# NVIDIA/nv-wavenet

Hardware: AMD Instinct MI355X
Metric: samples/sec (all GPUs) in real time (every utterance >= 24 kHz) and max real-time batch @24kHz, R64/S256/A256 20L fp16 (higher is better)
Workload: dtype f16; 1 GPU; C3: R=64 S=256 A=256 L=20 maxDilation=512 fp16, autoregressive generation at steady state (each step = samples 640..895 of every utterance: all dilated taps live, all rings wrapped; the steps re-run that sample range -- same launch, same memory traffic -- so from the second step on the rings hold the previous step's values: a timing workload, not one long utterance); batch_per_gpu=12288, global_batch=12288, parallelism=batch-sharded x1, final RCCL all_gather

## Files before the change

### nv_wavenet_amd/csrc/wn_kernels.hpp

```cpp
#pragma once

#include <hip/hip_runtime.h>
#include <utility>
#include <stdint.h>

#include <type_traits>

#include "wn_experiments.hpp"

namespace wn {

#define WN_DEV __device__ __forceinline__

typedef _Float16 half8 __attribute__((ext_vector_type(8)));
typedef _Float16 half4 __attribute__((ext_vector_type(4)));
typedef float floatx4 __attribute__((ext_vector_type(4)));
typedef unsigned int uintx4 __attribute__((ext_vector_type(4)));
typedef unsigned int uintx2 __attribute__((ext_vector_type(2)));

template <bool F16> struct Prec;
template <> struct Prec<true> {
    using elem = _Float16;
    using frag = half8;
    using quad = half4;
// ... 579 lines not shown

WN_DEV float fma_mix_lo(unsigned h2, float acc) {
    float d;
    asm("v_fma_mix_f32 %0, %1, 1.0, %2 op_sel_hi:[1,0,0]" : "=v"(d) : "v"(h2), "v"(acc));
    return d;
}
WN_DEV float fma_mix_hi(unsigned h2, float acc) {
    float d;
    asm("v_fma_mix_f32 %0, %1, 1.0, %2 op_sel:[1,0,0] op_sel_hi:[1,0,0]" : "=v"(d) : "v"(h2), "v"(acc));
    return d;
}
template <bool F16> WN_DEV void cond_add(floatx4* a, typename Prec<F16>::frag c, const typename Prec<F16>::frag* selA) {
    if constexpr (F16) {
#if WN_COND_VALU
        (void)selA;
        const uintx4 q = __builtin_bit_cast(uintx4, c);
        a[0][0] = fma_mix_lo(q[0], a[0][0]);
        a[0][1] = fma_mix_hi(q[0], a[0][1]);
        a[0][2] = fma_mix_lo(q[1], a[0][2]);
        a[0][3] = fma_mix_hi(q[1], a[0][3]);
        a[1][0] = fma_mix_lo(q[2], a[1][0]);
        a[1][1] = fma_mix_hi(q[2], a[1][1]);
        a[1][2] = fma_mix_lo(q[3], a[1][2]);
        a[1][3] = fma_mix_hi(q[3], a[1][3]);
#else
#pragma unroll
        for (int tt = 0; tt < Prec<F16>::TPF; tt++) a[tt] = mma(selA[tt], c, a[tt]);
#endif
    } else {
        (void)selA;
#pragma unroll
        for (int e = 0; e < Prec<F16>::EPL; e++) a[e >> 2][e & 3] += (float)c[e];
    }
}

template <bool F16, int R, int S, int A, int BT, bool EMBLDS, bool DUMP = true, int RAW = 0, bool LR = false>
#ifdef WN_EXP_TWO_WG
__global__ __launch_bounds__((Cfg<F16, R, S, A, BT>::THREADS), (BT == 1 ? 2 : 1)) void wavenet_wg(const Params p) {
#else
__global__ __launch_bounds__((Cfg<F16, R, S, A, BT>::THREADS), 1) void wavenet_wg(const Params p) {
#endif
    constexpr bool FEAT = RAW == 3;
    constexpr int KFC = FEAT ? feat_kfc<F16>() : 0;
    using C = Cfg<F16, R, S, A, BT, KFC>;
    using P = Prec<F16>;
    using frag = typename P::frag;
    using quad = typename P::quad;
    using elem = typename P::elem;
    constexpr int PF = C::PF, FLW = C::FLW, FHW = C::FHW, NW = C::NW;
    constexpr int RT = C::RT, HTW = C::HTW, STW = C::STW, ATW = C::ATW;
    constexpr int KF_R = C::KF_R, KF_S = C::KF_S, KF_A = C::KF_A;

    extern __shared__ __attribute__((aligned(16))) char lds[];
    char* const xbuf = lds + C::OFF_X;
    char* const hbuf = lds + C::OFF_H;
    char* const skbuf = lds + C::OFF_SK;
    char* const zsbuf = lds + C::OFF_ZS;
    float* const lgbuf = (float*)(lds + C::OFF_LG);
    int* const ybuf = (int*)(lds + C::OFF_Y);
    char* const xpbuf = lds + C::OFF_XP;
    float* const biasLds = (float*)(lds + C::OFF_BIAS);

    static_assert(RAW == 0 || RAW == 1 || (RAW == 2 && F16) || RAW == 3, "RAW: 0 packed, 1 fp32 in place, 2 fp16 in place (fp16 engine), 3 features");
    if (p.gate != nullptr && __builtin_nontemporal_load(p.gate) == 0u) return;

    const int tid = threadIdx.x;
    const int lane = tid & 63;
    const int w = __builtin_amdgcn_readfirstlane(tid >> 6);
    const int g = lane >> 4, j = lane & 15;
    const int L = p.numLayers;
    const int tile0 = p.tileBase + blockIdx.x * BT;
    if (p.clk != nullptr && blockIdx.x == 0 && tid == 0) {
        p.clk[0] = __builtin_amdgcn_s_memtime();
        p.clk[1] = __builtin_amdgcn_s_memrealtime();
    }

    int ub[BT];
    bool uvalid[BT];
#pragma unroll
    for (int bt = 0; bt < BT; bt++) {
        const int b = (tile0 + bt) * 16 + j;
        uvalid[bt] = b < p.batch;
        ub[bt] = uvalid[bt] ? b : p.batch - 1;
    }
    const int su = tid / C::LPU, sq = tid % C::LPU;

    constexpr int BLS = DUMP ? C::BIAS_L : C::BIAS_LN;
    if constexpr (DUMP) {
        const int nb = L * C::BIAS_L + 2 * A;
        for (int i = tid; i < nb; i += C::THREADS) biasLds[i] = p.bias[i];
        __syncthreads();
        for (int s0 = tid; s0 < S; s0 += C::THREADS) {
            float run = biasLds[3 * R + s0];
            for (int l = 1; l < L; l++) {
                run += biasLds[l * C::BIAS_L + 3 * R + s0];
                biasLds[l * C::BIAS_L + 3 * R + s0] = run;
            }
        }
    } else {
        for (int i = tid; i < L * C::BIAS_LN; i += C::THREADS) biasLds[i] = p.bias[(i / C::BIAS_LN) * C::BIAS_L + i % C::BIAS_LN];
        for (int i = tid; i < 2 * A; i += C::THREADS) biasLds[L * C::BIAS_LN + S + i] = p.bias[L * C::BIAS_L + i];
        for (int s0 = tid; s0 < S; s0 += C::THREADS) {
            float run = p.bias[3 * R + s0];
            for (int l = 1; l < L; l++) run += p.bias[l * C::BIAS_L + 3 * R + s0];
            biasLds[L * C::BIAS_LN + s0] = run;
        }
    }
    const float* const skipBiasSum = DUMP ? biasLds + (L - 1) * C::BIAS_L + 3 * R : biasLds + L * C::BIAS_LN;
    const float* const headBias = biasLds + (C::biasFloats(L, DUMP) - 2 * A);

    const unsigned laneOff = (unsigned)lane * 16u;
    const char* const wbase = (const char*)p.wblob + (size_t)w * C::waveStreamFrags(L) * 1024;
    const char* const whead = wbase + C::headOffsetFrags(L) * 1024;
    const elem* embPrev = (const elem*)p.embPrev;
    const elem* embCur = (const elem*)p.embCur;
    if constexpr (EMBLDS) {
        elem* const embLds = (elem*)(biasLds + C::biasFloats(L, DUMP));
        const floatx4* s0 = (const floatx4*)p.embCur;
        const floatx4* s1 = (const floatx4*)p.embPrev;
        constexpr int CH = (int)(A * R * sizeof(elem) / 16);
        for (int i = tid; i < CH; i += C::THREADS) {
            ((floatx4*)embLds)[i] = s0[i];
            if (p.embLds > 1) ((floatx4*)embLds)[CH + i] = s1[i];
        }
        embCur = embLds;
        if (p.embLds > 1) embPrev = embLds + A * R;
        __syncthreads();
    }

    int yPrev[BT], yCur[BT];
    floatx4 ep[BT][HTW];
#pragma unroll
    for (int bt = 0; bt < BT; bt++) {
        yPrev[bt] = p.yInPrev[ub[bt]];
        yCur[bt] = p.yInCur[ub[bt]];
#pragma unroll
        for (int i = 0; i < HTW; i++)
            ep[bt][i] = quad_to_f32(*(const quad*)(embPrev + (size_t)yPrev[bt] * R + (w + NW * i) * 16 + g * 4));
    }

    constexpr bool ws_pin = F16 && !(RAW == 1 && BT == 2);
    WStream<F16, PF, ws_pin> ws;
    const rsrc_t rsW = make_rsrc(wbase);
#pragma unroll
    for (int i = 0; i < PF; i++) ws.buf[i] = buf_load<frag, WN_W_AUX>(rsW, laneOff + (unsigned)(i & 3) * 1024u, (unsigned)(i & ~3) * 1024u);

    constexpr int HR = C::HR, HS = C::HS;
    frag hw[HR ? HR : 1];
    if constexpr (HR > 0) {
#pragma unroll
        for (int i = 0; i < HR; i++) hw[i] = *(const frag*)(whead + (size_t)C::headFrag(HS + i) * 1024 + laneOff);
    }

    constexpr int XPW = C::XPW;
    frag xpA[BT][XPW], xpB[BT][XPW];
    constexpr int CR = (RAW == 1 && F16) ? 2 * C::COND_FR : C::COND_FR;
    frag cdA[BT][CR], cdB[BT][CR];
    constexpr int KFCR = FEAT ? KFC : 1;
    frag cfCur[BT][KFCR], cfNext[BT][KFCR];
    const size_t featStride = (size_t)p.tiles * KFC * 1024;
    const char* const featMine = (const char*)p.feat + (size_t)tile0 * KFC * 1024;
    auto load_feat = [&](int tn, frag (&dst)[BT][KFCR]) {
        const int tc = tn < p.condSamples ? tn : p.condSamples - 1;
        const rsrc_t rsF = make_rsrc(featMine + (size_t)tc * featStride);
#pragma unroll
        for (int bt = 0; bt < BT; bt++)
#pragma unroll
            for (int k = 0; k < KFC; k++)
                dst[bt][k] = buf_load<frag, WN_FEAT_AUX>(rsF, laneOff + (unsigned)(k & 3) * 1024u, (unsigned)((bt * KFC + (k & ~3)) * 1024));
    };
    const size_t condStride = (size_t)p.tiles * NW * C::COND_FR * 1024;
    const char* const condMine = (const char*)p.cond + ((size_t)tile0 * NW + w) * C::COND_FR * 1024;
    const size_t ringTile = (size_t)p.ringSlots * KF_R * 1024;
    char* const ringMine = (char*)p.ring + (size_t)tile0 * ringTile;
    const rsrc_t rsRing = make_rsrc(ringMine);
    const unsigned ringTileB = (unsigned)ringTile;
    const int ldsD = LR ? p.ldsRingD : 0;
    char* const ringLds = lds + C::ringSlotOffset(0, (int)C::ldsBytes(L, EMBLDS ? p.embLds : 0, DUMP));
    const char* condNext = condMine + (size_t)p.initSample * L * condStride;
    constexpr unsigned RAWE = RAW == 2 ? 2u : 4u;
    const size_t rawRow = (size_t)p.maxBatch * (2 * R) * RAWE;
    unsigned rawOff[BT];
#pragma unroll
    for (int bt = 0; bt < BT; bt++) rawOff[bt] = ((unsigned)ub[bt] * (unsigned)(2 * R) + (unsigned)g * 4u) * RAWE;
    auto prefetch = [&](int tn, int ln, Dil dl, frag (&xd)[BT][XPW], frag (&cdd)[BT][CR]) {
        if (ln >= L) { ln -= L; tn += 1; }
        const unsigned slot = (unsigned)(dl.off + (tn & (dl.d - 1)));
        const unsigned rp0 = slot * (unsigned)(KF_R * 1024);
        const rsrc_t rsCond = make_rsrc(condNext);
        condNext += condStride;
        if (dl.d > ldsD) {
#pragma unroll
            for (int i = 0; i < XPW; i++) {
                const int k = w + NW * i;
                if (k < KF_R) {
#pragma unroll
                    for (int bt = 0; bt < BT; bt++)
                        xd[bt][i] = buf_load<frag, WN_RING_LD_AUX>(rsRing, laneOff, rp0 + (unsigned)bt * ringTileB + (unsigned)k * 1024u);
                }
            }
        }
#pragma unroll
        for (int bt = 0; bt < BT; bt++) {
            if constexpr (FEAT) {
            } else if constexpr (RAW != 0) {
                const int tc = tn < p.condSamples ? tn : p.condSamples - 1;
                const rsrc_t rsRaw = make_rsrc((const char*)p.condRaw + ((size_t)tc * L + ln) * rawRow);
                auto slotOff = [&](int it) { return (unsigned)((w + NW * (it >> 1) + (it & 1) * RT) * 16) * RAWE; };
                if constexpr (RAW == 1) {
#pragma unroll
                    for (int it = 0; it < 2 * HTW; it++) cdd[bt][it] = buf_load<frag, WN_RAW_AUX>(rsRaw, rawOff[bt], slotOff(it));
                } else {
#pragma unroll
                    for (int k = 0; k < HTW; k++) {
                        const uintx2 qa = __builtin_amdgcn_raw_buffer_load_b64(rsRaw, rawOff[bt], slotOff(2 * k), WN_RAW_AUX);
                        const uintx2 qb = __builtin_amdgcn_raw_buffer_load_b64(rsRaw, rawOff[bt], slotOff(2 * k + 1), WN_RAW_AUX);
                        cdd[bt][k] = __builtin_bit_cast(frag, uintx4{qa[0], qa[1], qb[0], qb[1]});
                    }
                }
            } else {
#pragma unroll
                for (int k = 0; k < C::COND_FR; k++)
                    cdd[bt][k] = buf_load<frag, WN_COND_AUX>(rsCond, laneOff + (unsigned)(k & 3) * 1024u,
                                                   (unsigned)((bt * NW * C::COND_FR + (k & ~3)) * 1024));
            }
        }
    };
    auto ring_lds_copy = [&](auto TOLDS) {
        constexpr bool toLds = decltype(TOLDS)::value;
        if (ldsD <= 0) return;
        Dil dl = dil_first();
        for (int l = 0; l < L; l++) {
            if (dl.d <= ldsD) {
                const int rows = dl.d * BT * KF_R;
                for (int r = w; r < rows; r += NW) {
                    const int sl = r / (BT * KF_R), bt = (r / KF_R) % BT, k = r % KF_R;
                    const unsigned hb = (unsigned)(dl.off + sl) * (unsigned)(KF_R * 1024) + (unsigned)bt * ringTileB + (unsigned)k * 1024u;
                    char* const lp = ringLds + (size_t)(dl.lds + sl) * C::RING_SLOT + ((bt * KF_R + k) * 64 + lane) * 16;
                    if constexpr (toLds) *(frag*)lp = buf_load<frag, WN_RING_LD_AUX>(rsRing, laneOff, hb);
                    else buf_store<frag, WN_RING_ST_AUX>(rsRing, laneOff, hb, *(const frag*)lp);
                }
            }
            dl = dil_next(dl, p.maxDilation, false, ldsD);
        }
    };
    ring_lds_copy(std::true_type{});
    prefetch(p.initSample, 0, p.dil[0], xpA, cdA);
    prefetch(p.initSample, 1, p.dil[1], xpB, cdB);
    auto publish_xp = [&](const frag (&xpN)[BT][XPW], const Dil dN) {
        if (dN.d <= ldsD) return;
#pragma unroll
        for (int i = 0; i < XPW; i++) {
            const int k = w + NW * i;
            if (k < KF_R) {
#pragma unroll
                for (int bt = 0; bt < BT; bt++) *(frag*)(xpbuf + ((bt * KF_R + k) * 64 + lane) * 16) = xpN[bt][i];
            }
        }
    };
    auto tap_image = [&](const Dil dN, int tn) -> const char* {
        return dN.d <= ldsD ? ringLds + (size_t)(dN.lds + (tn & (dN.d - 1))) * C::RING_SLOT : xpbuf;
    };
    publish_xp(xpA, p.dil[0]);

    __syncthreads();

#ifdef WN_TIMING
    unsigned long long tacc[12] = {0};
    unsigned long long tmark = 0;
#define WN_TMARK(i)                                                        \
    {                                                                      \
        unsigned long long _n = __builtin_amdgcn_s_memtime();              \
        asm volatile("s_waitcnt lgkmcnt(0)" ::: "memory");                 \
        tacc[i] += _n - tmark;                                             \
        tmark = _n;                                                        \
    }
#else
#define WN_TMARK(i)
#endif
    frag selA[P::TPF];
#pragma unroll
    for (int tt = 0; tt < P::TPF; tt++)
#pragma unroll
        for (int e = 0; e < P::EPL; e++)
            selA[tt][e] = (elem)(((e >> 2) == tt && g * 4 + (e & 3) == j) ? 1.0f : 0.0f);
    floatx4 acc[BT][2 * HTW];
    {
        frag xp[BT][KF_R];
#pragma unroll
        for (int bt = 0; bt < BT; bt++) {
            lds_get_frags<F16, KF_R>(tap_image(p.dil[0], p.initSample) + bt * KF_R * 1024, lane, xp[bt]);
#pragma unroll
            for (int i = 0; i < HTW; i++) {
                acc[bt][2 * i] = *(const floatx4*)(biasLds + (w + NW * i) * 16 + g * 4);
                acc[bt][2 * i + 1] = *(const floatx4*)(biasLds + (w + NW * i + RT) * 16 + g * 4);
            }
        }
        if constexpr (FEAT) {
            load_feat(p.initSample, cfNext);
#pragma unroll
            for (int bt = 0; bt < BT; bt++)
#pragma unroll
                for (int k = 0; k < KFC; k++) cfCur[bt][k] = agpr_operand<F16>(cfNext[bt][k]);
            gemm_direct<F16, BT, 2 * HTW, KFC>(wbase + C::streamPos(0, C::O_COND, L) * 1024, laneOff, acc, cfCur);
            load_feat(p.initSample + 1, cfNext);
#pragma unroll
            for (int bt = 0; bt < BT; bt++)
#pragma unroll
                for (int k = 0; k < KFC; k++) asm volatile("" ::"v"(cfNext[bt][k]));
        } else {
#pragma unroll
            for (int bt = 0; bt < BT; bt++)
#pragma unroll
                for (int k = 0; k < C::COND_FR; k++) cond_add<F16>(&acc[bt][k * P::TPF], cond_frag<F16, RAW>(cdA[bt], k), selA);
        }
        gemm_direct<F16, BT, 2 * HTW, KF_R>(wbase + C::streamPos(0, C::O_PREV, L) * 1024, laneOff, acc, xp);
    }
    float sscale[FEAT ? BT : 1];
    if constexpr (FEAT) {
#pragma unroll
        for (int bt = 0; bt < BT; bt++) {
            int sb = (tile0 + bt) * 16 + su;
            sb = sb < p.batch ? sb : p.batch - 1;
            sscale[bt] = p.softScale != nullptr ? p.softScale[sb] : kLog2e;
        }
    }
    const int tEnd = p.initSample + p.count;
    for (int t = p.initSample; t < tEnd; t++) {
        const bool dumpNow = DUMP && p.dump && (t == tEnd - 1);

        float selv[BT];
        if (!p.useRng) {
#pragma unroll
            for (int bt = 0; bt < BT; bt++) {
                int sb = (tile0 + bt) * 16 + su;
                sb = sb < p.batch ? sb : p.batch - 1;
                selv[bt] = p.sel[(size_t)t * p.maxBatch + sb];
            }
        }

        WN_TMARK(11)
        floatx4 x[BT][HTW];
#pragma unroll
        for (int bt = 0; bt < BT; bt++) {
#pragma unroll
            for (int i = 0; i < HTW; i++) {
                const int tile = w + NW * i;
                floatx4 ec = quad_to_f32(*(const quad*)(embCur + (size_t)yCur[bt] * R + tile * 16 + g * 4));
                floatx4 v = ep[bt][i] + ec;
                if (p.tanhEmbed) {
#pragma unroll
                    for (int r = 0; r < 4; r++) v[r] = tanh_t<F16>(v[r]);
                }
                x[bt][i] = v;
                lds_put_tile<F16>(xbuf + bt * KF_R * 1024, tile, lane, v);
            }
#pragma unroll
            for (int i = 0; i < HTW; i++)
                ep[bt][i] = quad_to_f32(*(const quad*)(embPrev + (size_t)yCur[bt] * R + (w + NW * i) * 16 + g * 4));
        }
        wg_barrier();
        WN_TMARK(0)

        floatx4 skip[BT][STW];
#pragma unroll
        for (int bt = 0; bt < BT; bt++)
#pragma unroll
            for (int i = 0; i < STW; i++) skip[bt][i] = floatx4{0.f, 0.f, 0.f, 0.f};

        frag hb[BT][KF_R];
        frag xb[BT][KF_R];
#pragma unroll
        for (int bt = 0; bt < BT; bt++) lds_get_frags<F16, KF_R>(xbuf + bt * KF_R * 1024, lane, xb[bt]);
        auto layer = [&](auto withSkip, const int l, const Dil dl, const Dil dN, const Dil dl2, frag (&xpC)[BT][XPW],
                         frag (&cdC)[BT][CR], const frag (&xpN)[BT][XPW], const frag (&cdN)[BT][CR]) {
            constexpr bool SKIP = decltype(withSkip)::value;
            constexpr int PB = SKIP ? 0 : FLW;
            const int wl = SKIP ? (l - 1) * FLW : 0;
            const float* bl = biasLds + l * BLS;
            const int lN = l + 1 < L ? l + 1 : 0;
            const float* blN = biasLds + lN * BLS;
            const int d = dl.d;

            WN_TMARK(1)
            gemm_b<F16, PF, 0, BT, 2 * HTW, KF_R>(ws, rsW, SKIP ? C::P_CUR : C::P_CUR0 - PB, wl, 0, laneOff, acc, xb);
            const bool ringInLds = d <= ldsD;
            frag xkeep[BT][XPW];
            if (!ringInLds) {
                const unsigned rp = (unsigned)(dl.off + (t & (d - 1))) * (unsigned)(KF_R * 1024);
#pragma unroll
                for (int k = 0; k < KF_R; k++)
                    if (k % NW == w) {
#pragma unroll
                        for (int bt = 0; bt < BT; bt++)
                            buf_store<frag, WN_RING_ST_AUX>(rsRing, laneOff + (unsigned)(k & 3) * 1024u,
                                               rp + (unsigned)bt * ringTileB + (unsigned)(k & ~3) * 1024u, xb[bt][k]);
                    }
            } else {
#pragma unroll
                for (int k = 0; k < KF_R; k++)
                    if (k % NW == w) {
#pragma unroll
                        for (int bt = 0; bt < BT; bt++) xkeep[bt][k / NW] = xb[bt][k];
                    }
            }
            if constexpr (!SKIP) prefetch(t, l + 2, dl2, xpC, cdC);
            __builtin_amdgcn_sched_barrier(0);
            WN_TMARK(2)

            floatx4 accN[FEAT ? BT : 1][2 * HTW];
            if constexpr (FEAT) {
#pragma unroll
                for (int bt = 0; bt < BT; bt++)
#pragma unroll
                    for (int i = 0; i < HTW; i++) {
                        accN[bt][2 * i] = *(const floatx4*)(blN + (w + NW * i) * 16 + g * 4);
                        accN[bt][2 * i + 1] = *(const floatx4*)(blN + (w + NW * i + RT) * 16 + g * 4);
                    }
            }
            if constexpr (FEAT) {
                constexpr int NS = BT * HTW * 2 * 5;
                constexpr int NFS = SKIP ? STW * KF_R : 0, NFC = C::FW_COND;
                constexpr int NM = (NFS + NFC) * BT;
                constexpr int G0S = STW >= 4 ? 4 : STW, G0C = 2 * HTW >= 4 ? 4 : 2 * HTW;
                constexpr bool EARLY = PF > 1;
                floatx2 ea, eb, ra, rb, hp;
                floatx4 hv;
                auto stage = [&](auto SI) {
                    constexpr int s = decltype(SI)::value, pr = s / 5, st = s % 5;
                    constexpr int bt = pr / (2 * HTW), i = (pr / 2) % HTW, r = (pr & 1) * 2;
                    gate_stage<F16, st>(acc[bt][2 * i][r], acc[bt][2 * i][r + 1], acc[bt][2 * i + 1][r], acc[bt][2 * i + 1][r + 1],
                                        ea, eb, ra, rb, hp);
                    if constexpr (st == 4) {
                        hv[r] = hp[0];
                        hv[r + 1] = hp[1];
                        if constexpr (r == 2) lds_put_tile<F16>(hbuf + bt * KF_R * 1024, w + NW * i, lane, hv);
                    }
                    __builtin_amdgcn_sched_barrier(0);
                };
                static_for<NFS + NFC>([&](auto FI) {
                    constexpr int fi = decltype(FI)::value;
                    constexpr bool isSkip = fi < NFS;
                    constexpr int q = isSkip ? fi : fi - NFS, G0 = isSkip ? G0S : G0C, KFq = isSkip ? KF_R : KFC;
                    constexpr int kf = (q / G0) % KFq, mt = (q / (G0 * KFq)) * G0 + q % G0;
                    constexpr int pos = isSkip ? C::P_SKIP + q : C::P_COND - PB + q;
                    constexpr int posPrev = (fi - 1 < NFS) ? C::P_SKIP + fi - 1 : C::P_COND - PB + fi - 1 - NFS;
                    frag a[1];
                    take_group<F16, PF, ws_pin, 1>(ws, pos, a);
                    if constexpr (EARLY && fi > 0) refill_group<F16, PF, 0, ws_pin, 1>(ws, rsW, posPrev, wl, 0, laneOff);
                    static_for<BT>([&](auto BI) {
                        constexpr int bt = decltype(BI)::value, m = fi * BT + bt;
                        if constexpr (isSkip) skip[bt][mt] = mma(a[0], hb[bt][kf], skip[bt][mt]);
                        else accN[bt][mt] = mma(a[0], cfCur[bt][kf], accN[bt][mt]);
                        __builtin_amdgcn_sched_barrier(0);
                        static_for_range<m * NS / NM, (m + 1) * NS / NM>(stage);
                    });
                    if constexpr (!EARLY || fi == NFS + NFC - 1) refill_group<F16, PF, 0, ws_pin, 1>(ws, rsW, pos, wl, 0, laneOff);
                    if constexpr (SKIP && fi == (NFS + NFC) * WN_REQ_AT_FEAT / 8) {
                        prefetch(t, l + 2, dl2, xpC, cdC);
                        __builtin_amdgcn_sched_barrier(0);
                    }
                });
                if (l == L - 2) {
                    asm volatile("");
#pragma unroll
                    for (int bt = 0; bt < BT; bt++)
#pragma unroll
                        for (int k = 0; k < KFC; k++) cfCur[bt][k] = agpr_operand<F16>(cfNext[bt][k]);
                }
                if constexpr (SKIP) {
                    if (dumpNow) {
                        const float* bp = biasLds + (l - 1) * C::BIAS_L + 3 * R;
#pragma unroll
                        for (int bt = 0; bt < BT; bt++) {
                            if (!uvalid[bt]) continue;
#pragma unroll
                            for (int i = 0; i < STW; i++)
                                *(floatx4*)(p.skipOut + ((size_t)(l - 1) * p.maxBatch + ub[bt]) * S + (w + NW * i) * 16 + g * 4) =
                                    skip[bt][i] + *(const floatx4*)(bp + (w + NW * i) * 16 + g * 4);
                        }
                    }
                }
            } else {
                constexpr int NS = BT * HTW * 2 * 5;
                constexpr int NM = SKIP ? STW * KF_R * BT : 0;
                floatx2 ea, eb, ra, rb, hp;
                floatx4 hv;
                auto stage = [&](auto SI) {
                    constexpr int s = decltype(SI)::value, pr = s / 5, st = s % 5;
                    constexpr int bt = pr / (2 * HTW), i = (pr / 2) % HTW, r = (pr & 1) * 2;
                    gate_stage<F16, st>(acc[bt][2 * i][r], acc[bt][2 * i][r + 1], acc[bt][2 * i + 1][r], acc[bt][2 * i + 1][r + 1],
                                        ea, eb, ra, rb, hp);
                    if constexpr (st == 4) {
                        hv[r] = hp[0];
                        hv[r + 1] = hp[1];
                        if constexpr (r == 2) lds_put_tile<F16>(hbuf + bt * KF_R * 1024, w + NW * i, lane, hv);
                    }
                    __builtin_amdgcn_sched_barrier(0);
                };
                if constexpr (SKIP) {
                    constexpr int G0 = STW >= 4 ? 4 : STW, G = take_g(G0, PF);
                    static_for<STW * KF_R / G>([&](auto GI) {
                        constexpr int gi = decltype(GI)::value, q = gi * G;
                        constexpr int kf = (q / G0) % KF_R, mg = q / (G0 * KF_R), mi0 = q % G0;
                        frag a[G];
                        take_group<F16, PF, ws_pin, G>(ws, C::P_SKIP + gi * G, a);
                        constexpr bool EARLY = PF > G;
                        if constexpr (EARLY && gi > 0) refill_group<F16, PF, 0, ws_pin, G>(ws, rsW, C::P_SKIP + (gi - 1) * G, wl, 0, laneOff);
                        static_for<G * BT>([&](auto MI) {
                            constexpr int mi = decltype(MI)::value / BT, bt = decltype(MI)::value % BT;
                            constexpr int mt = mg * G0 + mi0 + mi, m = (q + mi) * BT + bt;
                            skip[bt][mt] = mma(a[mi], hb[bt][kf], skip[bt][mt]);
                            __builtin_amdgcn_sched_barrier(0);
                            static_for_range<m * NS / NM, (m + 1) * NS / NM>(stage);
                        });
                        if constexpr (!EARLY || gi == STW * KF_R / G - 1) refill_group<F16, PF, 0, ws_pin, G>(ws, rsW, C::P_SKIP + gi * G, wl, 0, laneOff);
                        if constexpr (gi == (STW * KF_R / G) * WN_REQ_AT / 8) {
                            prefetch(t, l + 2, dl2, xpC, cdC);
                            __builtin_amdgcn_sched_barrier(0);
                        }
                    });
                    if (dumpNow) {
                        const float* bp = biasLds + (l - 1) * C::BIAS_L + 3 * R;
#pragma unroll
                        for (int bt = 0; bt < BT; bt++) {
                            if (!uvalid[bt]) continue;
#pragma unroll
                            for (int i = 0; i < STW; i++)
                                *(floatx4*)(p.skipOut + ((size_t)(l - 1) * p.maxBatch + ub[bt]) * S + (w + NW * i) * 16 + g * 4) =
                                    skip[bt][i] + *(const floatx4*)(bp + (w + NW * i) * 16 + g * 4);
                        }
                    }
                } else {
                    static_for<NS>(stage);
                }
            }
            WN_TMARK(3)
            wg_barrier();
            WN_TMARK(4)
#pragma unroll
            for (int bt = 0; bt < BT; bt++) lds_get_frags<F16, KF_R>(hbuf + bt * KF_R * 1024, lane, hb[bt]);
            if (ringInLds) {
                char* const sl = ringLds + (size_t)(dl.lds + (t & (d - 1))) * C::RING_SLOT;
#pragma unroll
                for (int i = 0; i < XPW; i++) {
                    const int k = w + NW * i;
                    if (k < KF_R) {
#pragma unroll
                        for (int bt = 0; bt < BT; bt++) *(frag*)(sl + ((bt * KF_R + k) * 64 + lane) * 16) = xkeep[bt][i];
                    }
                }
            }

            floatx4 xa[BT][HTW];
#pragma unroll
            for (int bt = 0; bt < BT; bt++)
#pragma unroll
                for (int i = 0; i < HTW; i++)
                    xa[bt][i] = *(const floatx4*)(bl + 2 * R + (w + NW * i) * 16 + g * 4) + x[bt][i];
#pragma unroll
            for (int bt = 0; bt < BT; bt++)
#pragma unroll
                for (int i = 0; i < HTW; i++) {
                    if constexpr (FEAT) {
                        acc[bt][2 * i] = accN[bt][2 * i];
                        acc[bt][2 * i + 1] = accN[bt][2 * i + 1];
                    } else {
                        acc[bt][2 * i] = *(const floatx4*)(blN + (w + NW * i) * 16 + g * 4);
                        acc[bt][2 * i + 1] = *(const floatx4*)(blN + (w + NW * i + RT) * 16 + g * 4);
                    }
                }

            gemm_b<F16, PF, 0, BT, HTW, KF_R>(ws, rsW, C::P_RES - PB, wl, 0, laneOff, xa, hb);
#pragma unroll
            for (int bt = 0; bt < BT; bt++)
#pragma unroll
                for (int i = 0; i < HTW; i++) {
                    x[bt][i] = xa[bt][i];
                    lds_put_tile<F16>(xbuf + bt * KF_R * 1024, w + NW * i, lane, xa[bt][i]);
                }
            publish_xp(xpN, dN);
            __builtin_amdgcn_sched_barrier(0);
            WN_TMARK(5)
            if constexpr (FEAT) {
            } else {
#pragma unroll
                for (int bt = 0; bt < BT; bt++)
#pragma unroll
                    for (int k = 0; k < C::COND_FR; k++) cond_add<F16>(&acc[bt][k * P::TPF], cond_frag<F16, RAW>(cdN[bt], k), selA);
            }
            if (dumpNow) {
#pragma unroll
                for (int bt = 0; bt < BT; bt++) {
                    if (!uvalid[bt]) continue;
#pragma unroll
                    for (int i = 0; i < HTW; i++)
                        *(floatx4*)(p.xtOut + ((size_t)l * p.maxBatch + ub[bt]) * R + (w + NW * i) * 16 + g * 4) = x[bt][i];
                }
            }
            __builtin_amdgcn_sched_barrier(0);
            WN_TMARK(6)
            wg_barrier();
            WN_TMARK(7)
            frag xp[BT][KF_R];
            const char* const tapImg = tap_image(dN, l + 1 < L ? t : t + 1);
#pragma unroll
            for (int bt = 0; bt < BT; bt++) lds_get_frags<F16, KF_R>(tapImg + bt * KF_R * 1024, lane, xp[bt]);
#pragma unroll
            for (int bt = 0; bt < BT; bt++) lds_get_frags<F16, KF_R>(xbuf + bt * KF_R * 1024, lane, xb[bt]);
            __builtin_amdgcn_sched_barrier(0);
            gemm_b<F16, PF, 0, BT, 2 * HTW, KF_R>(ws, rsW, C::P_PREV - PB, wl, 0, laneOff, acc, xp);
        };
        {
            Dil da = dil_first(), db = dil_next(da, p.maxDilation, L == 1, ldsD), dc = dil_next(db, p.maxDilation, L == 2, ldsD);
            auto adv = [&](int l) { da = db; db = dc; dc = dil_next(dc, p.maxDilation, l + 3 == L, ldsD); };
            layer(std::false_type{}, 0, da, db, dc, xpA, cdA, xpB, cdB);
            adv(0);
            int l = 1;
            for (; l + 1 < L; l += 2) {
                layer(std::true_type{}, l, da, db, dc, xpB, cdB, xpA, cdA);
                adv(l);
                layer(std::true_type{}, l + 1, da, db, dc, xpA, cdA, xpB, cdB);
                adv(l + 1);
            }
            if (l < L) layer(std::true_type{}, l, da, db, dc, xpB, cdB, xpA, cdA);
            if (L & 1) {
#pragma unroll
                for (int bt = 0; bt < BT; bt++) {
#pragma unroll
                    for (int i = 0; i < XPW; i++) {
                        const frag tmp = xpA[bt][i];
                        xpA[bt][i] = xpB[bt][i];
                        xpB[bt][i] = tmp;
                    }
#pragma unroll
                    for (int k = 0; k < CR; k++) {
                        const frag tmp = cdA[bt][k];
                        cdA[bt][k] = cdB[bt][k];
                        cdB[bt][k] = tmp;
                    }
                }
            }
        }
        gemm_b<F16, PF, 0, BT, STW, KF_R>(ws, rsW, C::P_CUR, (L - 1) * FLW, 0, laneOff, skip, hb);

#pragma unroll
        for (int bt = 0; bt < BT; bt++)
#pragma unroll
            for (int i = 0; i < STW; i++) {
                floatx4 v = skip[bt][i] + *(const floatx4*)(skipBiasSum + (w + NW * i) * 16 + g * 4);
#pragma unroll
                for (int r = 0; r < 4; r++) v[r] = __builtin_fmaxf(v[r], 0.f);
                lds_put_tile<F16>(skbuf + bt * KF_S * 1024, w + NW * i, lane, v);
                if (dumpNow && uvalid[bt])
                    *(floatx4*)(p.skipOut + ((size_t)(L - 1) * p.maxBatch + ub[bt]) * S + (w + NW * i) * 16 + g * 4) = v;
            }
        wg_barrier();
        floatx4 zs[BT][ATW];
        if constexpr (HS != 0 && KF_S * BT * 4 > WN_ZS_B_REGS) {
#pragma unroll
            for (int bt = 0; bt < BT; bt++)
#pragma unroll
                for (int i = 0; i < ATW; i++) zs[bt][i] = *(const floatx4*)(headBias + (w + NW * i) * 16 + g * 4);
            gemm_ldsb_b<F16, PF, C::HSP, BT, ATW, KF_S>(ws, rsW, C::O_ZS, L * FLW, 0, laneOff, zs, skbuf, lane);
            skip_frags<F16, PF, C::HSP, ws_pin, C::PAD1>(ws, rsW, C::FW_ZS, L * FLW, 0, laneOff);
        } else {
            frag sb[BT][KF_S];
#pragma unroll
            for (int bt = 0; bt < BT; bt++) {
                lds_get_frags<F16, KF_S>(skbuf + bt * KF_S * 1024, lane, sb[bt]);
#pragma unroll
                for (int i = 0; i < ATW; i++) zs[bt][i] = *(const floatx4*)(headBias + (w + NW * i) * 16 + g * 4);
            }
            if constexpr (HS == 0) gemm_res<F16, BT, ATW, KF_S>(hw, 0, zs, sb);
            else {
                gemm_b<F16, PF, C::HSP, BT, ATW, KF_S>(ws, rsW, C::O_ZS, L * FLW, 0, laneOff, zs, sb);
                skip_frags<F16, PF, C::HSP, ws_pin, C::PAD1>(ws, rsW, C::FW_ZS, L * FLW, 0, laneOff);
            }
        }
#pragma unroll
        for (int bt = 0; bt < BT; bt++)
#pragma unroll
            for (int i = 0; i < ATW; i++) {
#pragma unroll
                for (int r = 0; r < 4; r++) zs[bt][i][r] = __builtin_fmaxf(zs[bt][i][r], 0.f);
                lds_put_tile<F16>(zsbuf + bt * KF_A * 1024, w + NW * i, lane, zs[bt][i]);
                if (dumpNow && uvalid[bt])
                    *(floatx4*)(p.zs + (size_t)ub[bt] * A + (w + NW * i) * 16 + g * 4) = zs[bt][i];
            }
        wg_barrier();
        floatx4 za[BT][ATW];
        {
#pragma unroll
            for (int bt = 0; bt < BT; bt++)
#pragma unroll
                for (int i = 0; i < ATW; i++)
                    za[bt][i] = *(const floatx4*)(headBias + A + (w + NW * i) * 16 + g * 4);
            auto draw_selectors = [&]() {
                if (!p.useRng) return;
                if constexpr (C::LPU == 16 && BT > 1) {
                    const int q = sq < BT ? sq : 0;
                    int sb = (tile0 + q) * 16 + su;
                    sb = sb < p.batch ? sb : p.batch - 1;
                    const float mine = philox_selector(p.rngKey0, p.rngKey1, (unsigned)t, (unsigned)sb);
                    selv[0] = dpp_f<0x150>(mine);
                    if constexpr (BT > 1) selv[1] = dpp_f<0x151>(mine);
                    if constexpr (BT > 2) selv[2] = dpp_f<0x152>(mine);
                    if constexpr (BT > 3) selv[3] = dpp_f<0x153>(mine);
                } else {
#pragma unroll
                    for (int bt = 0; bt < BT; bt++) {
                        int sb = (tile0 + bt) * 16 + su;
                        sb = sb < p.batch ? sb : p.batch - 1;
                        selv[bt] = philox_selector(p.rngKey0, p.rngKey1, (unsigned)t, (unsigned)sb);
                    }
                }
            };
            if constexpr (C::ZA_B_FROM_LDS) {
                static_assert(HR == 0, "the LDS-streamed head is for the large, non-resident heads");
                draw_selectors();
                gemm_ldsb_b<F16, PF, C::HSP, BT, ATW, KF_A>(ws, rsW, C::O_ZA, L * FLW, 0, laneOff, za, zsbuf, lane);
            } else {
                frag zb[BT][KF_A];
#pragma unroll
                for (int bt = 0; bt < BT; bt++) lds_get_frags<F16, KF_A>(zsbuf + bt * KF_A * 1024, lane, zb[bt]);
                draw_selectors();
                if constexpr (HR >= C::FW_ZA) gemm_res<F16, BT, ATW, KF_A>(hw, C::FW_ZS - HS, za, zb);
                else gemm_b<F16, PF, C::HSP, BT, ATW, KF_A>(ws, rsW, C::O_ZA, L * FLW, 0, laneOff, za, zb);
            }
        }
        if constexpr (C::ALIAS_LG) wg_barrier();
        constexpr int LGT = C::LGT;
        auto put_logits = [&](auto PASS) {
            constexpr int pass = decltype(PASS)::value;
#pragma unroll
            for (int bl = 0; bl < LGT; bl++)
#pragma unroll
                for (int i = 0; i < ATW; i++) {
                    const int bt = pass * LGT + bl;
                    *(floatx4*)(lgbuf + (bl * 16 + j) * C::LROW + (w + NW * i) * 16 + g * 4) = za[bt][i];
                    if (dumpNow && uvalid[bt])
                        *(floatx4*)(p.za + (size_t)ub[bt] * A + (w + NW * i) * 16 + g * 4) = za[bt][i];
                }
        };
        put_logits(std::integral_constant<int, 0>{});
        WN_TMARK(8)
        if constexpr (HS == FHW) {
            skip_frags<F16, PF, C::HSP, ws_pin, C::PAD2>(ws, rsW, C::O_ZA + C::FW_ZA, L * FLW, 0, laneOff);
        }
        if constexpr (FEAT) load_feat(t + 2, cfNext);
        wg_barrier();
        WN_TMARK(9)

        static_for<BT / LGT>([&](auto PASS) {
            constexpr int pass = decltype(PASS)::value;
            if constexpr (pass > 0) {
                wg_barrier();
                put_logits(PASS);
                wg_barrier();
            }
#pragma unroll
            for (int bl = 0; bl < LGT; bl++) {
                const int bt = pass * LGT + bl;
                float e[C::RPL];
                float total;
                const float* lrow = lgbuf + (bl * 16 + su) * C::LROW + sq * C::RPL;
                int pick;
                if constexpr (FEAT) pick = softmax_pick<A, C::LPU, C::RPL>(lrow, sq, lane, selv[bt], e, total, sscale[bt]);
                else pick = softmax_pick<A, C::LPU, C::RPL>(lrow, sq, lane, selv[bt], e, total);
                const int sb = (tile0 + bt) * 16 + su;
                if (sq == 0) {
                    ybuf[bt * 16 + su] = pick;
                    if (sb < p.batch) p.yOut[(size_t)sb * p.numSamples + t] = pick;
                }
                if (dumpNow && sb < p.batch) {
                    const float inv = 1.0f / total;
#pragma unroll
                    for (int i = 0; i < C::RPL / 4; i++)
                        *(floatx4*)(p.p + (size_t)sb * A + sq * C::RPL + i * 4) =
                            floatx4{e[i * 4] * inv, e[i * 4 + 1] * inv, e[i * 4 + 2] * inv, e[i * 4 + 3] * inv};
                }
            }
        });
        wg_barrier();
#pragma unroll
        for (int bt = 0; bt < BT; bt++) {
            yPrev[bt] = yCur[bt];
// ... 343 lines not shown
```

Before: 328.7 million samples/s.

## Restructure dilation ring bookkeeping into per-wave row ownership with precomputed ring entries

Replaces the per-layer Dil slot arithmetic with a RingEnt struct that precomputes the slot offset, LDS tap pointer and whether the ring lives in LDS. Each wave now owns whole rows across the batch tiles (NROW = BT*KF_R spread over waves) for prefetch, publish and ring store. For small R the ring store and load always go through a buffer resource whose record count is zero when the ring is LDS-resident, which removes branches but issues masked global ops. Own rows are read back from xbuf instead of being kept in registers, trading register pressure for extra LDS reads.

Result: no change. 330.4 million samples/s, median of 6 (+0.5%).

```diff
diff --git a/nv_wavenet_amd/csrc/wn_kernels.hpp b/nv_wavenet_amd/csrc/wn_kernels.hpp
--- a/nv_wavenet_amd/csrc/wn_kernels.hpp
+++ b/nv_wavenet_amd/csrc/wn_kernels.hpp
@@ -755,8 +755,11 @@
         for (int i = 0; i < HR; i++) hw[i] = *(const frag*)(whead + (size_t)C::headFrag(HS + i) * 1024 + laneOff);
     }
 
-    constexpr int XPW = C::XPW;
-    frag xpA[BT][XPW], xpB[BT][XPW];
+    constexpr int NROW = BT * KF_R, RPW = (NROW + NW - 1) / NW;
+    constexpr bool OWN_EARLY = R <= 128;
+    constexpr unsigned ROWB = (unsigned)(KF_R * 1024);
+    const bool lastRow = NROW % NW == 0 || w + NW * (RPW - 1) < NROW;
+    frag xpA[RPW], xpB[RPW];
     constexpr int CR = (RAW == 1 && F16) ? 2 * C::COND_FR : C::COND_FR;
     frag cdA[BT][CR], cdB[BT][CR];
     constexpr int KFCR = FEAT ? KFC : 1;
@@ -779,29 +782,62 @@
     const rsrc_t rsRing = make_rsrc(ringMine);
     const unsigned ringTileB = (unsigned)ringTile;
     const int ldsD = LR ? p.ldsRingD : 0;
-    char* const ringLds = lds + C::ringSlotOffset(0, (int)C::ldsBytes(L, EMBLDS ? p.embLds : 0, DUMP));
+    const unsigned ringLdsOff = (unsigned)C::ringSlotOffset(0, (int)C::ldsBytes(L, EMBLDS ? p.embLds : 0, DUMP));
+    char* const ringLds = lds + ringLdsOff;
+    const unsigned rowLds = (unsigned)w * 1024u + laneOff;
+    unsigned rowHbm[RPW];
+#pragma unroll
+    for (int i = 0; i < RPW; i++) {
+        const int r = w + NW * i;
+        rowHbm[i] = BT == 1 ? rowLds : laneOff + (unsigned)(r / KF_R) * ringTileB + (unsigned)(r % KF_R) * 1024u;
+    }
+    auto row_soff = [&](unsigned slot, int i) { return BT == 1 ? slot + (unsigned)(i * NW * 1024) : slot; };
+    struct RingEnt {
+        int mask;
+        unsigned hbm;
+        char* ldsAcc;
+        int far;
+        unsigned slot;
+        char* tap;
+        WN_DEV bool inLds() const { return LR && far < 0; }
+        WN_DEV int records() const { return LR ? ~(far >> 31) : -1; }
+    };
+    auto ring_rsrc = [&](const RingEnt e) { return __builtin_amdgcn_make_buffer_rsrc((void*)ringMine, 0, e.records(), 0x00020000); };
+    auto ent_make = [&](int d, unsigned hbm, char* ldsAcc, int tn) {
+        RingEnt e;
+        e.mask = d - 1, e.hbm = hbm, e.ldsAcc = ldsAcc;
+        e.far = e.mask - ldsD;
+        const unsigned ph = (unsigned)(tn & e.mask);
+        e.slot = hbm + ph * ROWB;
+        e.tap = e.inLds() ? ldsAcc + ph * (unsigned)C::RING_SLOT : xpbuf;
+        return e;
+    };
+    auto ent_first = [&](int tn) { return ent_make(1, 0u, ringLds, tn); };
+    auto ent_next = [&](const RingEnt s, int rel, int t0) {
+        const bool toFirst = rel == 0;
+        const int sd = s.mask + 1;
+        int d = toFirst ? 0x40000000 : sd << 1;
+        const unsigned hbm = toFirst ? 0u : s.hbm + (unsigned)sd * ROWB;
+        char* const acc = toFirst ? ringLds : s.ldsAcc + (unsigned)(s.inLds() ? sd : 0) * (unsigned)C::RING_SLOT;
+        const int tn = t0 + 1 + (rel >> 31);
+        if (d > p.maxDilation) d = 1;
+        return ent_make(d, hbm, acc, tn);
+    };
     const char* condNext = condMine + (size_t)p.initSample * L * condStride;
     constexpr unsigned RAWE = RAW == 2 ? 2u : 4u;
     const size_t rawRow = (size_t)p.maxBatch * (2 * R) * RAWE;
     unsigned rawOff[BT];
 #pragma unroll
     for (int bt = 0; bt < BT; bt++) rawOff[bt] = ((unsigned)ub[bt] * (unsigned)(2 * R) + (unsigned)g * 4u) * RAWE;
-    auto prefetch = [&](int tn, int ln, Dil dl, frag (&xd)[BT][XPW], frag (&cdd)[BT][CR]) {
+    auto prefetch = [&](int tn, int ln, const RingEnt dl, frag (&xd)[RPW], frag (&cdd)[BT][CR]) {
         if (ln >= L) { ln -= L; tn += 1; }
-        const unsigned slot = (unsigned)(dl.off + (tn & (dl.d - 1)));
-        const unsigned rp0 = slot * (unsigned)(KF_R * 1024);
         const rsrc_t rsCond = make_rsrc(condNext);
         condNext += condStride;
-        if (dl.d > ldsD) {
-#pragma unroll
-            for (int i = 0; i < XPW; i++) {
-                const int k = w + NW * i;
-                if (k < KF_R) {
-#pragma unroll
-                    for (int bt = 0; bt < BT; bt++)
-                        xd[bt][i] = buf_load<frag, WN_RING_LD_AUX>(rsRing, laneOff, rp0 + (unsigned)bt * ringTileB + (unsigned)k * 1024u);
-                }
-            }
+        if (OWN_EARLY || !dl.inLds()) {
+            const rsrc_t rs = OWN_EARLY ? ring_rsrc(dl) : rsRing;
+#pragma unroll
+            for (int i = 0; i < RPW; i++)
+                if (i + 1 < RPW || lastRow) xd[i] = buf_load<frag, WN_RING_LD_AUX>(rs, rowHbm[i], row_soff(dl.slot, i));
         }
 #pragma unroll
         for (int bt = 0; bt < BT; bt++) {
@@ -848,23 +884,16 @@
         }
     };
     ring_lds_copy(std::true_type{});
-    prefetch(p.initSample, 0, p.dil[0], xpA, cdA);
-    prefetch(p.initSample, 1, p.dil[1], xpB, cdB);
-    auto publish_xp = [&](const frag (&xpN)[BT][XPW], const Dil dN) {
-        if (dN.d <= ldsD) return;
-#pragma unroll
-        for (int i = 0; i < XPW; i++) {
-            const int k = w + NW * i;
-            if (k < KF_R) {
-#pragma unroll
-                for (int bt = 0; bt < BT; bt++) *(frag*)(xpbuf + ((bt * KF_R + k) * 64 + lane) * 16) = xpN[bt][i];
-            }
-        }
+    prefetch(p.initSample, 0, ent_first(p.initSample), xpA, cdA);
+    prefetch(p.initSample, 1, ent_next(ent_first(p.initSample), 1 - L, p.initSample), xpB, cdB);
+    auto publish_xp = [&](const frag (&xpN)[RPW], const RingEnt dN) {
+        if (dN.inLds()) return;
+#pragma unroll
+        for (int i = 0; i < RPW; i++)
+            if (i + 1 < RPW || lastRow) *(frag*)(xpbuf + rowLds + i * NW * 1024) = xpN[i];
     };
-    auto tap_image = [&](const Dil dN, int tn) -> const char* {
-        return dN.d <= ldsD ? ringLds + (size_t)(dN.lds + (tn & (dN.d - 1))) * C::RING_SLOT : xpbuf;
-    };
-    publish_xp(xpA, p.dil[0]);
+    auto tap_image = [&](const RingEnt dN) -> const char* { return dN.tap; };
+    publish_xp(xpA, ent_first(p.initSample));
 
     __syncthreads();
 
@@ -892,7 +921,7 @@
         frag xp[BT][KF_R];
 #pragma unroll
         for (int bt = 0; bt < BT; bt++) {
-            lds_get_frags<F16, KF_R>(tap_image(p.dil[0], p.initSample) + bt * KF_R * 1024, lane, xp[bt]);
+            lds_get_frags<F16, KF_R>(tap_image(ent_first(p.initSample)) + bt * KF_R * 1024, lane, xp[bt]);
 #pragma unroll
             for (int i = 0; i < HTW; i++) {
                 acc[bt][2 * i] = *(const floatx4*)(biasLds + (w + NW * i) * 16 + g * 4);
@@ -975,37 +1004,35 @@
         frag xb[BT][KF_R];
 #pragma unroll
         for (int bt = 0; bt < BT; bt++) lds_get_frags<F16, KF_R>(xbuf + bt * KF_R * 1024, lane, xb[bt]);
-        auto layer = [&](auto withSkip, const int l, const Dil dl, const Dil dN, const Dil dl2, frag (&xpC)[BT][XPW],
-                         frag (&cdC)[BT][CR], const frag (&xpN)[BT][XPW], const frag (&cdN)[BT][CR]) {
+        static_assert(OWN_EARLY || (BT == 1 && KF_R % NW == 0), "rows of a wave = its fragments of xb");
+        frag xo[RPW];
+        auto get_own_rows = [&]() {
+#pragma unroll
+            for (int i = 0; i < RPW; i++) xo[i] = *(const frag*)(xbuf + rowLds + i * NW * 1024);
+        };
+        if constexpr (OWN_EARLY) get_own_rows();
+        auto layer = [&](auto withSkip, const int l, const RingEnt dl, const RingEnt dN, const RingEnt dl2, frag (&xpC)[RPW],
+                         frag (&cdC)[BT][CR], const frag (&xpN)[RPW], const frag (&cdN)[BT][CR]) {
             constexpr bool SKIP = decltype(withSkip)::value;
             constexpr int PB = SKIP ? 0 : FLW;
             const int wl = SKIP ? (l - 1) * FLW : 0;
             const float* bl = biasLds + l * BLS;
             const int lN = l + 1 < L ? l + 1 : 0;
             const float* blN = biasLds + lN * BLS;
-            const int d = dl.d;
 
             WN_TMARK(1)
             gemm_b<F16, PF, 0, BT, 2 * HTW, KF_R>(ws, rsW, SKIP ? C::P_CUR : C::P_CUR0 - PB, wl, 0, laneOff, acc, xb);
-            const bool ringInLds = d <= ldsD;
-            frag xkeep[BT][XPW];
-            if (!ringInLds) {
-                const unsigned rp = (unsigned)(dl.off + (t & (d - 1))) * (unsigned)(KF_R * 1024);
-#pragma unroll
-                for (int k = 0; k < KF_R; k++)
-                    if (k % NW == w) {
-#pragma unroll
-                        for (int bt = 0; bt < BT; bt++)
-                            buf_store<frag, WN_RING_ST_AUX>(rsRing, laneOff + (unsigned)(k & 3) * 1024u,
-                                               rp + (unsigned)bt * ringTileB + (unsigned)(k & ~3) * 1024u, xb[bt][k]);
-                    }
-            } else {
-#pragma unroll
-                for (int k = 0; k < KF_R; k++)
-                    if (k % NW == w) {
-#pragma unroll
-                        for (int bt = 0; bt < BT; bt++) xkeep[bt][k / NW] = xb[bt][k];
-                    }
+            if (OWN_EARLY || !dl.inLds()) {
+                const rsrc_t rs = OWN_EARLY ? ring_rsrc(dl) : rsRing;
+                if constexpr (OWN_EARLY) {
+#pragma unroll
+                    for (int i = 0; i < RPW; i++)
+                        if (i + 1 < RPW || lastRow) buf_store<frag, WN_RING_ST_AUX>(rs, rowHbm[i], row_soff(dl.slot, i), xo[i]);
+                } else {
+#pragma unroll
+                    for (int k = 0; k < KF_R; k++)
+                        if (k % NW == w) buf_store<frag, WN_RING_ST_AUX>(rs, laneOff, dl.slot + (unsigned)k * 1024u, xb[0][k]);
+                }
             }
             if constexpr (!SKIP) prefetch(t, l + 2, dl2, xpC, cdC);
             __builtin_amdgcn_sched_barrier(0);
@@ -1143,16 +1170,12 @@
             WN_TMARK(4)
 #pragma unroll
             for (int bt = 0; bt < BT; bt++) lds_get_frags<F16, KF_R>(hbuf + bt * KF_R * 1024, lane, hb[bt]);
-            if (ringInLds) {
-                char* const sl = ringLds + (size_t)(dl.lds + (t & (d - 1))) * C::RING_SLOT;
-#pragma unroll
-                for (int i = 0; i < XPW; i++) {
-                    const int k = w + NW * i;
-                    if (k < KF_R) {
-#pragma unroll
-                        for (int bt = 0; bt < BT; bt++) *(frag*)(sl + ((bt * KF_R + k) * 64 + lane) * 16) = xkeep[bt][i];
-                    }
-                }
+            if (dl.inLds()) {
+                if constexpr (!OWN_EARLY) get_own_rows();
+                char* const sl = dl.tap;
+#pragma unroll
+                for (int i = 0; i < RPW; i++)
+                    if (i + 1 < RPW || lastRow) *(frag*)(sl + rowLds + i * NW * 1024) = xo[i];
             }
 
             floatx4 xa[BT][HTW];
@@ -1206,17 +1229,18 @@
             wg_barrier();
             WN_TMARK(7)
             frag xp[BT][KF_R];
-            const char* const tapImg = tap_image(dN, l + 1 < L ? t : t + 1);
+            const char* const tapImg = tap_image(dN);
 #pragma unroll
             for (int bt = 0; bt < BT; bt++) lds_get_frags<F16, KF_R>(tapImg + bt * KF_R * 1024, lane, xp[bt]);
 #pragma unroll
             for (int bt = 0; bt < BT; bt++) lds_get_frags<F16, KF_R>(xbuf + bt * KF_R * 1024, lane, xb[bt]);
+            if constexpr (OWN_EARLY) get_own_rows();
             __builtin_amdgcn_sched_barrier(0);
             gemm_b<F16, PF, 0, BT, 2 * HTW, KF_R>(ws, rsW, C::P_PREV - PB, wl, 0, laneOff, acc, xp);
         };
         {
-            Dil da = dil_first(), db = dil_next(da, p.maxDilation, L == 1, ldsD), dc = dil_next(db, p.maxDilation, L == 2, ldsD);
-            auto adv = [&](int l) { da = db; db = dc; dc = dil_next(dc, p.maxDilation, l + 3 == L, ldsD); };
+            RingEnt da = ent_first(t), db = ent_next(da, 1 - L, t), dc = ent_next(db, 2 - L, t);
+            auto adv = [&](int l) { da = db; db = dc; dc = ent_next(dc, l + 3 - L, t); };
             layer(std::false_type{}, 0, da, db, dc, xpA, cdA, xpB, cdB);
             adv(0);
             int l = 1;
@@ -1229,13 +1253,13 @@
             if (l < L) layer(std::true_type{}, l, da, db, dc, xpB, cdB, xpA, cdA);
             if (L & 1) {
 #pragma unroll
+                for (int i = 0; i < RPW; i++) {
+                    const frag tmp = xpA[i];
+                    xpA[i] = xpB[i];
+                    xpB[i] = tmp;
+                }
+#pragma unroll
                 for (int bt = 0; bt < BT; bt++) {
-#pragma unroll
-                    for (int i = 0; i < XPW; i++) {
-                        const frag tmp = xpA[bt][i];
-                        xpA[bt][i] = xpB[bt][i];
-                        xpB[bt][i] = tmp;
-                    }
 #pragma unroll
                     for (int k = 0; k < CR; k++) {
                         const frag tmp = cdA[bt][k];
```
